# laurabragagnolo/SkelSplat

Hardware: AMD Instinct MI355X
Metric: rendered+backpropagated views/s (differentiable skeletal-Gaussian rasterizer fwd+bwd) (higher is better)
Workload: dtype f32

## Files before the change

include/skelsplat_hip.h:

```cpp
#ifndef SKELSPLAT_HIP_H
#define SKELSPLAT_HIP_H

#include <stddef.h>
#include <stdint.h>

#ifdef __cplusplus
extern "C" {
#endif

#define SKS_MAX_VIEWS 64
#define SKS_MAX_CHANNELS 32
#define SKS_SMALL_P 256

#define SKS_ANTIALIASING 1u
#define SKS_CLAMP01      2u
#define SKS_FORCE_BINNED 4u
#define SKS_DEBUG_SYNC   8u

#define SKS_NO_NT_STORES 16u

#define SKS_RAW_PARAMS   32u
#define SKS_RAW_GRADS    128u
#define SKS_BIN_CLEAN    64u
#define SKS_BIN_GROUPS_SHIFT 16
#define SKS_BIN_GROUPS(n) ((unsigned)(((n) - 1) & 7) << SKS_BIN_GROUPS_SHIFT)
#define SKS_FILL_LINEAR (1u << 21)
#define SKS_FILL_ROWS (1u << 22)
#define SKS_BWD_LDS_LIST (1u << 20)
#define SKS_BWD_WG_SHIFT 23

const char* sks_last_error(void);
int sks_version(void);

int sks_scratch_bytes(int V, int P, int C, int W, int H, size_t bin_capacity,
                      size_t* geom_bytes, size_t* binning_bytes, size_t* accum_bytes);

int sks_forward(int V, int P, int C, int W, int H,
                const float* viewmatrix, const float* projmatrix,
                const float* tanfovx , const float* tanfovy ,
                const float* means3D, const float* features, const float* opacities,
                const float* scales, const float* rotations, const float* cov3D_precomp,
                float scale_modifier, unsigned flags,
                float* out_color, float* out_invdepth, int* radii,
                void* geom, void* binning, size_t bin_capacity, int* num_rendered_dev,
                float* final_T, uint32_t* n_contrib, void* stream);

int sks_backward(int V, int P, int C, int W, int H,
                 const float* viewmatrix, const float* projmatrix,
                 const float* tanfovx , const float* tanfovy ,
                 const float* bg,
// ... 143 lines not shown
```

skelsplat_amd/_lib.py:

```python
import ctypes as C
import os

_HERE = os.path.dirname(os.path.abspath(__file__))
LIB_PATH = os.path.join(_HERE, "libskelsplat_hip.so")
_lib = None

SKS_MAX_VIEWS = 64
SKS_MAX_CHANNELS = 32
SKS_SMALL_P = 256
SKS_ANTIALIASING = 1
SKS_CLAMP01 = 2
SKS_FORCE_BINNED = 4
SKS_DEBUG_SYNC = 8
SKS_NO_NT_STORES = 16
SKS_RAW_PARAMS = 32
SKS_BIN_CLEAN = 64
SKS_RAW_GRADS = 128
SKS_FB_NO_JOIN = 1
SKS_BIN_GROUPS_SHIFT = 16
SKS_SSIM_SCRATCH_BYTES = 64 * 8


def SKS_BIN_GROUPS(n):
    return ((int(n) - 1) & 7) << SKS_BIN_GROUPS_SHIFT
# ... 32 lines not shown
    "sks_backward_fused_loss": (_i, [_i, _i, _i, _i, _i, _vp, _vp, _vp, _vp, _vp, _vp, _vp, _vp, _vp, _vp, _vp, _f, _u,
                                     _vp, _vp, _vp, _vp, _vp, _vp, _vp, _vp, _vp, _vp, _vp, _vp, _vp, _vp, _vp, _vp, _vp, _vp, _vp]),
    "sks_loop_pack_grads": (_i, [_i, _i, _vp, _vp, _vp, _vp, _vp, _vp, _vp, _vp, _vp, _vp]),
    "sks_loop_adam_step": (_i, [_i, _i, _vp, _vp, C.c_ulonglong, _i, _vp, _vp, _vp, _vp, _vp, _vp, _vp, _i, _vp, _vp, _vp,
                                _f, _vp, _i, _vp]),
    "sks_loop_adam_step_es": (_i, [_i, _i, _vp, _vp, C.c_ulonglong, _i, _vp, _vp, _vp, _vp, _vp, _vp, _vp, _i, _vp, _vp, _vp,
                                   _f, _vp, _i, _vp, _vp, _i, _f, _vp, _vp]),
    "sks_loop_shard_floats": (_sz, [_i, _i, _i]),
    "sks_adam_multi": (_i, [_i, _vp, _vp, _vp, _vp, _vp, _vp, _vp, C.c_double, C.c_double, C.c_double, _vp]),
    "sks_loop_fused_step": (_i, [_i, _i, _i, _i, _i, _vp, _vp, _vp, _vp, _vp, _f, _u, _vp, _vp, _vp, _vp, _vp, _vp, _vp,
                                 _vp, C.c_ulonglong, _i, _vp, _vp, _vp, _vp, _vp, _vp, _vp, _i, _vp, _vp, _vp, _f, _vp, _vp, _vp,
                                 _i, _vp, _vp]),
    "sks_loop_fused_step_es": (_i, [_i, _i, _i, _i, _i, _vp, _vp, _vp, _vp, _vp, _f, _u, _vp, _vp, _vp, _vp, _vp, _vp, _vp,
                                    _vp, C.c_ulonglong, _i, _vp, _vp, _vp, _vp, _vp, _vp, _vp, _i, _vp, _vp, _vp, _f, _vp, _vp,
                                    _vp, _i, _vp, _vp, _i, _f, _vp, _vp]),
    "sks_prof_enable": (_i, [_i]),
    "sks_prof_spin": (_i, [C.c_double, _vp]),
    "sks_prof_read": (_i, [_i, C.POINTER(C.c_double), C.POINTER(C.c_longlong)]),
    "sks_prof_count": (_i, [_i, C.POINTER(C.c_longlong)]),
    "sks_prof_read_quantiles": (_i, [_i, C.POINTER(C.c_double), C.POINTER(C.c_double), C.POINTER(C.c_longlong)]),
}


def load(build_if_missing=True):
    global _lib
    if _lib is not None:
        return _lib
    if build_if_missing:
        try:
            from . import build as _b
# ... 62 lines not shown
```

skelsplat_amd/csrc/sks_bwd_small.inc:

```
template <int CG>
struct BwdPix {
    float T, T_final, last_alpha, accum_inv, last_inv, dLi, bgdot;
    float dL[CG], accum_rec[CG], last_color[CG];
};

struct BwdArgs {
    int P, C, W, H;
    unsigned flags;
    Geom g;
    const float* features;
    const float* bg;
    const float* dL_color;
    const float* dL_invdepth;
    float* accum;
    const float* tile_S;
    const float* tile_N;
    const float* hm_row = nullptr;
    const float* hm_col = nullptr;
    const float* hm_cmin = nullptr;
    const float* hm_den = nullptr;
    const int* es_stop = nullptr;
    int es_stride = 0;
    int es_views = 1;
};
// ... 489 lines not shown
        for (int j = 0; j < 8; j++) grp[j] = sum[j0 + j];
        const float r = wave_sum8(grp);
        if (lane < 8) s_red[buf][wv][j0 + lane] = r;
    }
#pragma unroll
    for (int j = NV & ~7; j < NV; j++) {
        const float r = wave_sum(sum[j]);
        if (lane == 0) s_red[buf][wv][j] = r;
    }
    __syncthreads();
    if (tid < NVS)
        out[tid * BWD_SPLITS] = tid < NV ? ((s_red[buf][0][tid] + s_red[buf][1][tid]) + (s_red[buf][2][tid] + s_red[buf][3][tid])) : 0.0f;
    }
}

__global__ __launch_bounds__(256) void k_gt_tile_stats(int C, int W, int H, const float* __restrict__ gt, float* __restrict__ tile_S,
                                                        float* __restrict__ tile_N, double* __restrict__ totals)
{
    __shared__ double s_t[2][4];
    const int band = blockIdx.x, ch = blockIdx.y, v = blockIdx.z, tid = threadIdx.x;
    const int gx = (W + TILE - 1) / TILE, gy = gridDim.x;
    const size_t HW = (size_t)H * W;
    const float* plane = gt + ((size_t)v * C + ch) * HW;
    const int y0 = band * TILE, rows = min(TILE, H - y0);
    const bool vec = (W & 3) == 0;
    double tS = 0.0, tN = 0.0;
    for (int t0 = 0; t0 < gx; t0 += 64) {
        const int tx = t0 + (tid >> 2), x = tx * TILE + (tid & 3) * 4;
        float S = 0.0f, N = 0.0f;
        if (tx < gx && x < W) {
// ... 41 lines not shown
```

skelsplat_amd/csrc/sks_common.inc:

```
thread_local char g_err[512] = "";

int fail(int code, const char* fmt, ...)
{
    va_list ap;
    va_start(ap, fmt);
    vsnprintf(g_err, sizeof(g_err), fmt, ap);
    va_end(ap);
    return code;
}

#define HIP_TRY(expr)                                                                          \
    do {                                                                                       \
        hipError_t e_ = (expr);                                                                \
        if (e_ != hipSuccess) return fail((int)e_, "%s: %s", #expr, hipGetErrorString(e_));    \
    } while (0)

#define STAGE_CHECK(name)                                                                      \
    do {                                                                                       \
        HIP_TRY(hipGetLastError());                                                            \
        if (flags & SKS_DEBUG_SYNC) {                                                          \
            hipError_t e_ = hipStreamSynchronize(st);                                          \
            if (e_ != hipSuccess) return fail((int)e_, "stage %s: %s", name, hipGetErrorString(e_)); \
        }                                                                                      \
    } while (0)
// ... 121 lines not shown
inline bool cover_per_plane(int P, int W, int H, int C)
{
    return cover_enabled(P, W, H) && (C + 1) * ((H + TILE - 1) / TILE) * cover_cw(W) <= COVER_MAX_WORDS;
}
inline Geom geom_from(void* base, int V, int P, int W, int H)
{
    char* p = (char*)base;
    Geom g;
    size_t n = (size_t)V * P;
    g.co = (float4*)p; p += align256(n * sizeof(float4));
    g.xyd = (float4*)p; p += align256(n * sizeof(float4));
    g.rect = (uint4*)p; p += align256(n * sizeof(uint4));
    g.cover = cover_enabled(P, W, H) ? (uint32_t*)p : nullptr;
    return g;
}
inline size_t geom_bytes(int V, int P, int W, int H, int C)
{
    const int planes = cover_per_plane(P, W, H, C) ? C + 1 : 1;
    return 3 * align256((size_t)V * P * 16) + align256((size_t)V * planes * ((H + TILE - 1) / TILE) * cover_cw(W) * 4);
}

constexpr int BIN_WAVE_SORT = 64;
constexpr int BIN_ROWS = 2;
constexpr int BIN_CLASSES = 8;
constexpr int BIN_HDR_CLASS = 8;
constexpr int BIN_MAX_GROUPS = 7;
#ifndef SKS_BIN_FB_GROUPS
#define SKS_BIN_FB_GROUPS 1
#endif
constexpr int BIN_FB_GROUPS = SKS_BIN_FB_GROUPS;
inline int bin_groups_default()
{
    static const int n = [] {
        const char* e = getenv("SKS_BIN_GROUPS");
// ... 68 lines not shown
```

skelsplat_amd/csrc/sks_geom_bwd.inc:

```
struct GeomBwdArgs {
    int P, C, W, H;
    unsigned flags;
    const float* vms;
    const float* pms;
    const float* means;
    const float* opac;
    const float* scales;
    const float* rots;
    const float* cov3Dp;
    float smod;
    const int* radii;
    const float* accum;
    int nsplit;
    const double* gt_totals;
    double* loss_sums;
    float* packed;
    float* dmeans3D;
    float* dmeans2D;
    float* dopacity;
    float* dscales;
    float* drots;
    float* dcov3D;
    float* dfeat;
    const uint4* rect = nullptr;
    const uint32_t* goff = nullptr;
    const float* part = nullptr;
    size_t cap = 0;
    const uint32_t* bin_hdr = nullptr;
    int v0 = 0;
};

__device__ __forceinline__ float sq(float x) { return x * x; }

__device__ __forceinline__ void geom_bwd_dfeat(const GeomBwdArgs& a, size_t o0, int n, int tid, int nthreads)
{
    const int ns = a.nsplit ? a.nsplit : 1, NVS = NACC + a.C;
    for (int e = tid; e < n * a.C; e += nthreads) {
        const int gi = e / a.C, ch = e - gi * a.C;
        const float* acc = a.accum + (o0 + gi) * ns * NVS + (size_t)(NACC + ch) * ns;
        float t = 0.0f;
        if (ns == BWD_SPLITS) {
            float4 q[4];
#pragma unroll
            for (int i = 0; i < 4; i++) q[i] = reinterpret_cast<const float4*>(acc)[i];
#pragma unroll
            for (int i = 0; i < 4; i++) { t += q[i].x; t += q[i].y; t += q[i].z; t += q[i].w; }
        } else {
            for (int sp = 0; sp < ns; sp++) t += acc[sp];
        }
        a.dfeat[(o0 + gi) * a.C + ch] = t;
    }
}

template <bool DFEAT_HERE = true>
__device__ __forceinline__ void geom_bwd_load(const GeomBwdArgs& a, int v, int idx, float (&g)[NACC], double& pS, double& pN)
{
    const size_t o = (size_t)v * a.P + (idx < a.P ? idx : 0);
    const int NVS = NACC + a.C;
    const float* acc = a.accum + o * (a.nsplit ? a.nsplit : 1) * NVS;
    if (a.nsplit == BWD_SPLITS) {
        static_assert(BWD_SPLITS == 16, "4 x float4 per value");
        float4 q[NACC][4];
#pragma unroll
        for (int j = 0; j < NACC - 1; j++)
#pragma unroll
            for (int i = 0; i < 4; i++) q[j][i] = reinterpret_cast<const float4*>(acc + j * BWD_SPLITS)[i];
#pragma unroll
        for (int j = 0; j < NACC - 1; j++) {
            float t = 0.0f;
#pragma unroll
            for (int i = 0; i < 4; i++) t += (q[j][i].x + q[j][i].y) + (q[j][i].z + q[j][i].w);
            g[j] = t;
        }
        g[NACC - 1] = 0.0f;
// ... 266 lines not shown
        if (raw) {
            const float so = 1.0f / (1.0f + expf_fixed(-(PRE ? pre->opac : a.opac[idx])));
            oj = so * (1.0f - so);
        }
        pk[10] = dop * oj * scl;
    }
}

__global__ __launch_bounds__(256) void k_geom_bwd(GeomBwdArgs a, ViewTan vt)
{
    const int idx = blockIdx.x * 256 + threadIdx.x;
    const int v = blockIdx.y;
    float g[NACC];
    double pS, pN;
    if (a.dfeat) geom_bwd_dfeat(a, (size_t)v * a.P + blockIdx.x * 256, min(256, a.P - (int)blockIdx.x * 256), threadIdx.x, 256);
    geom_bwd_load<false>(a, v, idx, g, pS, pN);
    double n_view = 1.0;
    if (a.loss_sums) {
        __shared__ double s_l[2][4];
        pS = wave_sum_d(pS);
        pN = wave_sum_d(pN);
        if ((threadIdx.x & 63) == 0) { s_l[0][threadIdx.x >> 6] = pS; s_l[1][threadIdx.x >> 6] = pN; }
        __syncthreads();
        const double S = a.gt_totals[2 * v] + ((s_l[0][0] + s_l[0][1]) + (s_l[0][2] + s_l[0][3]));
        n_view = a.gt_totals[2 * v + 1] + ((s_l[1][0] + s_l[1][1]) + (s_l[1][2] + s_l[1][3]));
        if (threadIdx.x == 0) {
            a.loss_sums[2 * v] = S;
            a.loss_sums[2 * v + 1] = n_view;
        }
    }
    if (idx >= a.P) return;
// ... 55 lines not shown
        const float* acc = a.accum + o * (NACC + a.C);
        for (int ch = 0; ch < a.C; ch++) a.dfeat[o * a.C + ch] = acc[NACC + ch];
    }
    geom_bwd_finish<true>(a, vt, v, idx, g, 1.0, &in);
}

__global__ __launch_bounds__(256) void k_geom_bwd_all(GeomBwdArgs a, ViewTan vt, int V, float* __restrict__ mean_out)
{
    const int t = threadIdx.x;
    const int v = t / a.P, idx = t - v * a.P;
    const bool live = v < V;
    float g[NACC];
    double pS, pN;
    if (a.dfeat) geom_bwd_dfeat(a, 0, V * a.P, t, 256);
    if (live) {
        geom_bwd_load<false>(a, v, idx, g, pS, pN);
        geom_bwd_finish(a, vt, v, idx, g, 1.0);
    }
    __syncthreads();
    if (t < a.P) {
        float m[3] = { 0.0f, 0.0f, 0.0f };
        for (int w0 = 0; w0 < V; w0 += 4) {
            float tv[4][3];
#pragma unroll
            for (int j = 0; j < 4; j++) {
                const float* gm = a.dmeans3D + ((size_t)(w0 + j < V ? w0 + j : V - 1) * a.P + t) * 3;
                tv[j][0] = gm[0]; tv[j][1] = gm[1]; tv[j][2] = gm[2];
            }
#pragma unroll
            for (int j = 0; j < 4; j++)
                if (w0 + j < V) { m[0] += tv[j][0]; m[1] += tv[j][1]; m[2] += tv[j][2]; }
// ... 93 lines not shown
```

skelsplat_amd/csrc/sks_geom_fwd.inc:

```
__device__ __forceinline__ uint4 geom_fwd_one(int P, const ViewTan& vt, const float* __restrict__ vms,
                                              const float* __restrict__ pms, const float* __restrict__ means,
                                              const float* __restrict__ opac, const float* __restrict__ scales,
                                              const float* __restrict__ rots, const float* __restrict__ cov3Dp,
                                              float smod, unsigned flags, const Geom& g, int* __restrict__ radii,
                                              int v, int idx, bool live, bool store = true)
{
    const size_t o = (size_t)v * P + (live ? idx : 0);
    const float* V = vms + 16 * v;
    const float* PM = pms + 16 * v;
    const float tan_fovx = vt.x[v], tan_fovy = vt.y[v];
    const int W = vt.w[v], H = vt.h[v];
    const float focal_y = H / (2.0f * tan_fovy);
    const float focal_x = W / (2.0f * tan_fovx);
    const int gx = (W + TILE - 1) / TILE, gy = (H + TILE - 1) / TILE;

    int radius_out = 0;
    uint4 rect = make_uint4(0, 0, 0, 0);
    float4 co = make_float4(0, 0, 0, 0), xyd = make_float4(0, 0, 1.0f, 1.0f);

    const int li = live ? idx : 0;
    const float p_orig[3] = { means[3 * li], means[3 * li + 1], means[3 * li + 2] };
    float p_view[3];
    transformPoint4x3(p_orig, V, p_view);
    if (live && p_view[2] > 0.2f) {
// ... 36 lines not shown
                radius_out = (int)my_radius;
                rect = make_uint4(xmin, ymin, xmax, ymax);
                const float op_raw = opac[li];
                const float op = (flags & SKS_RAW_PARAMS) ? 1.0f / (1.0f + expf_fixed(-op_raw)) : op_raw;
                co = make_float4(conic[0], conic[1], conic[2], op * h_convolution_scaling);
                xyd = make_float4(px, py, p_view[2], 1 / p_view[2]);
            }
        }
    }
    if (live && store) {
        radii[o] = radius_out;
        g.co[o] = co;
        g.xyd[o] = xyd;
        g.rect[o] = rect;
    }
    return rect;
}

#ifndef SKS_GEOM_COVER_THREADS
#define SKS_GEOM_COVER_THREADS 256
#endif
__global__ __launch_bounds__(SKS_GEOM_COVER_THREADS > 256 ? SKS_GEOM_COVER_THREADS : 256) void k_geom_fwd(int P, int W, int H, ViewTan vt, const float* __restrict__ vms,
                                                   const float* __restrict__ pms, const float* __restrict__ means,
                                                   const float* __restrict__ opac, const float* __restrict__ scales,
                                                   const float* __restrict__ rots, const float* __restrict__ cov3Dp,
                                                   float smod, unsigned flags, Geom g, int* __restrict__ radii, int vf,
                                                   uint32_t* __restrict__ count = nullptr, uint32_t* __restrict__ touched = nullptr,
                                                   const float* __restrict__ features = nullptr, int C = 0,
                                                   uint2* __restrict__ fmask = nullptr, uint32_t* __restrict__ bin_hdr = nullptr,
                                                   int cover_planes = 0)
{
    __shared__ uint32_t s_cov[COVER_MAX_WORDS];
    const int idx = blockIdx.x * blockDim.x + threadIdx.x;
    const int v = blockIdx.y;
    const bool live = idx < P;
    if (vf > 0) {
        const int fr = v / vf;
        means += (size_t)fr * P * 3;
        opac += (size_t)fr * P;
        if (scales) scales += (size_t)fr * P * 3;
        if (rots) rots += (size_t)fr * P * 4;
        if (cov3Dp) cov3Dp += (size_t)fr * P * 6;
    }
    const int pz = blockIdx.z;
    const uint4 rect = geom_fwd_one(P, vt, vms, pms, means, opac, scales, rots, cov3Dp, smod, flags, g, radii, v, idx, live, pz == 0);
    if (bin_hdr && blockIdx.x == 0 && blockIdx.y == 0 && pz == 0 && threadIdx.x < 64) bin_hdr[threadIdx.x] = 0u;
    if (count) {
        const int wt = (int)(rect.z - rect.x), n = wt * (int)(rect.w - rect.y);
        if (live) touched[(size_t)v * P + idx] = (uint32_t)n;
        if (live && v == 0) {
            unsigned fm = 0u;
            float f0 = 0.0f;
            for (int ch = C - 1; ch >= 0; ch--) {
                const float f = features[(size_t)idx * C + ch];
                if (f != 0.0f) { fm |= 1u << ch; f0 = f; }
            }
            fmask[idx] = make_uint2(fm, __float_as_uint(f0));
        }
    }
    if (g.cover) {
// ... 6 lines not shown
        if (mine) {
#pragma nounroll
            for (unsigned y = rect.y; y < rect.w; y++) {
                atomicOr(&s_cov[y * cw], 1u);
#pragma nounroll
                for (unsigned w0 = rect.x >> 5; w0 <= (rect.z - 1u) >> 5; w0++) {
                    const unsigned lo = max(rect.x, w0 << 5) & 31u, hi = min(rect.z - 1u, (w0 << 5) + 31u) & 31u;
                    atomicOr(&s_cov[y * cw + 1 + w0], (0xffffffffu >> (31u - hi)) & (0xffffffffu << lo));
                }
            }
        }
        __syncthreads();
        uint32_t* out = g.cover + ((size_t)v * (cover_planes ? C + 1 : 1) + (cover_planes ? pz : 0)) * pw;
        for (int i = threadIdx.x; i < pw; i += blockDim.x) out[i] = s_cov[i];
    }
}

__global__ void k_mark_visible(int P, const float* __restrict__ means, const float* __restrict__ V,
                               uint8_t* __restrict__ present)
{
    const int idx = blockIdx.x * 256 + threadIdx.x;
    if (idx >= P) return;
    const float p[3] = { means[3 * idx], means[3 * idx + 1], means[3 * idx + 2] };
    float pv[3];
    transformPoint4x3(p, V, pv);
    present[idx] = pv[2] > 0.2f;
}
```

skelsplat_amd/csrc/sks_raster.hip:

```cpp
#include <hip/hip_runtime.h>
#include <hip/hip_ext.h>
#include <stdarg.h>
#include <stdlib.h>
#include <stdio.h>
#include <string.h>

#include "../../include/skelsplat_hip.h"
#include "sks_math.h"
#include "sks_loop_dev.h"

using namespace sks;

namespace {

#include "sks_common.inc"
#include "sks_geom_fwd.inc"
#include "sks_fwd_small.inc"
#include "sks_bwd_small.inc"
#include "sks_geom_bwd.inc"
#include "sks_binned.inc"

inline int pick_cg(int C) { return C <= 4 ? 4 : C <= 16 ? 16 : C <= 20 ? 20 : 32; }

int check_common(int V, int P, int C, int W, int H)
// ... 105 lines not shown
            case 4: hipLaunchKernelGGL((k_render_bwd_wave<4, false, true, true, ES>), grid, dim3(256), 0, st, a, vt, vo); break;
            case 16: hipLaunchKernelGGL((k_render_bwd_wave<16, false, true, true, ES>), grid, dim3(256), 0, st, a, vt, vo); break;
            case 20: hipLaunchKernelGGL((k_render_bwd_wave<20, false, true, true, ES>), grid, dim3(256), 0, st, a, vt, vo); break;
            default: hipLaunchKernelGGL((k_render_bwd_wave<32, false, true, true, ES>), grid, dim3(256), 0, st, a, vt, vo); break;
        }
        return;
    }
    switch (cg) {
        case 4: hipLaunchKernelGGL((k_render_bwd_wave<4, false, true, false, ES>), grid, dim3(256), 0, st, a, vt, vo); break;
        case 16: hipLaunchKernelGGL((k_render_bwd_wave<16, false, true, false, ES>), grid, dim3(256), 0, st, a, vt, vo); break;
        case 20: hipLaunchKernelGGL((k_render_bwd_wave<20, false, true, false, ES>), grid, dim3(256), 0, st, a, vt, vo); break;
        default: hipLaunchKernelGGL((k_render_bwd_wave<32, false, true, false, ES>), grid, dim3(256), 0, st, a, vt, vo); break;
    }
}

template <int CG>
void launch_bwd_small(const BwdArgs& a, const ViewTan& vt, const ViewOff& vo, int V, int gy, bool dfeat, hipStream_t st,
                      const ProfScope& prof)
{
    (void)gy;
    if (a.P <= 64 && !(a.flags & (1u << 20))) {
        dim3 grid(a.P, V, bwd_wave_groups(V, a.P, a.flags));
        if (dfeat) SKS_LAUNCH(prof, (k_render_bwd_wave<CG, true, false>), grid, dim3(256), 0, st, a, vt, vo);
        else SKS_LAUNCH(prof, (k_render_bwd_wave<CG, false, false>), grid, dim3(256), 0, st, a, vt, vo);
        return;
    }
    dim3 grid(a.P, V, BWD_SPLITS);
    const size_t lds = GatherLds<CG>::bytes((a.P + 15) & ~15, CG, a.C);
    if (lds > 48 * 1024) {
        (void)hipFuncSetAttribute(reinterpret_cast<const void*>(&k_render_bwd_gather<CG, true>),
                                  hipFuncAttributeMaxDynamicSharedMemorySize, (int)lds);
        (void)hipFuncSetAttribute(reinterpret_cast<const void*>(&k_render_bwd_gather<CG, false>),
                                  hipFuncAttributeMaxDynamicSharedMemorySize, (int)lds);
    }
    if (dfeat) SKS_LAUNCH(prof, (k_render_bwd_gather<CG, true>), grid, dim3(256), lds, st, a);
// ... 46 lines not shown
}

}

#ifndef SKS_GEOM_BINNED_THREADS
#define SKS_GEOM_BINNED_THREADS 256
#endif

extern "C" {

const char* sks_last_error(void) { return g_err; }
void sks_set_error_(const char* msg)
{
    snprintf(g_err, sizeof(g_err), "%s", msg);
}
int sks_version(void) { return 12; }

int sks_scratch_bytes(int V, int P, int C, int W, int H, size_t bin_capacity, size_t* geom, size_t* binning, size_t* accum)
{
    if (int rc = check_common(V, P, C, W, H)) return rc;
    const int NT = ((W + TILE - 1) / TILE) * ((H + TILE - 1) / TILE);
    if (geom) *geom = geom_bytes(V, P > 0 ? P : 1, W, H, C);
    if (binning) *binning = bin_bytes(V, P, NT, bin_capacity, C + 1, (size_t)((H + TILE - 1) / TILE) * cover_cw(W));
    if (accum) *accum = (size_t)V * (P > 0 ? P : 1) * BWD_SPLITS * (NACC + C) * sizeof(float);
    return 0;
}

}

namespace {

int forward_impl(int V, int P, int C, int W, int H, const float* viewmatrix, const float* projmatrix,
                 const float* tanfovx, const float* tanfovy, const float* means3D, const float* features,
                 const float* opacities, const float* scales, const float* rotations, const float* cov3D_precomp,
                 float scale_modifier, unsigned flags, float* out_color, float* out_invdepth, int* radii, void* geom,
                 void* binning, size_t bin_capacity, int* num_rendered_dev, float* final_T, uint32_t* n_contrib,
                 void* stream, const FwdHook* hook)
{
    if (int rc = check_common(V, P, C, W, H)) return rc;
    hipStream_t st = (hipStream_t)stream;
// ... 18 lines not shown

    const bool small = P <= SKS_SMALL_P && !(flags & SKS_FORCE_BINNED);
    Bin b{};
    if (!small) {
        if (!binning) return fail(-2, "binned path needs a binning buffer");
        if (bin_capacity < 1) return fail(-1, "binned path needs bin_capacity >= 1");
        b = bin_from(binning, V, P, NT, bin_capacity);
    }
    if (!small) g.cover = nullptr;
    const int gthreads = small ? 256 : SKS_GEOM_BINNED_THREADS;
    const int gplanes = (small && g.cover && cover_per_plane(P, W, H, C)) ? C + 1 : 1;
    if (hook && small && hook->geom_done)
        hipExtLaunchKernelGGL(k_geom_fwd, dim3((P + gthreads - 1) / gthreads, V, gplanes), dim3(gthreads), 0, st, nullptr, hook->geom_done, 0,
                              P, W, H, vt, viewmatrix, projmatrix, means3D, opacities, scales, rotations, cov3D_precomp, scale_modifier,
                              flags, g, radii, 0, (uint32_t*)nullptr, (uint32_t*)nullptr, features, C, (uint2*)nullptr, (uint32_t*)nullptr,
                              cover_per_plane(P, W, H, C) ? 1 : 0);
    else
    hipLaunchKernelGGL(k_geom_fwd, dim3((P + gthreads - 1) / gthreads, V, gplanes), dim3(gthreads), 0, st, P, W, H, vt, viewmatrix, projmatrix,
                       means3D, opacities, scales, rotations, cov3D_precomp, scale_modifier, flags, g, radii, 0,
                       small ? (uint32_t*)nullptr : b.count, small ? (uint32_t*)nullptr : b.touched, features, C,
                       small ? (uint2*)nullptr : b.fmask, small ? (uint32_t*)nullptr : b.hdr, (small && cover_per_plane(P, W, H, C)) ? 1 : 0);
    STAGE_CHECK("geometry");
    if (hook && small && hook->after_geom) {
        if (int rc = hook->after_geom(hook->ctx)) return rc;
    }

    FwdArgs a{ P, C, W, H, flags, g, features, out_color, out_invdepth, final_T, n_contrib, composite_slots(flags, V, P),
               ((1u << 20) + (unsigned)C) / (unsigned)(C + 1), 0, (!small || (g.cover && cover_per_plane(P, W, H, C))) ? 1 : 0,
               (W >= 2 && W < 16384) ? (unsigned)(((1ull << 32) + (unsigned)W - 1) / (unsigned)W) : 0u };
    const int cg = pick_cg(C);
    if (small) {
        {
            ProfScope prof(0, st, true);
            switch (cg) {
                case 4: launch_fwd_small<4>(a, V, gy, st, prof); break;
                case 16: launch_fwd_small<16>(a, V, gy, st, prof); break;
// ... 84 lines not shown
    if (P == 0) return 0;
    hipStream_t st = (hipStream_t)stream;
    if (!viewmatrix || !projmatrix || !tanfovx || !tanfovy || !means3D || !features || !opacities || !radii ||
        !geom || !dL_dout_color || !accum || !dL_dmeans3D || !dL_dmeans2D || !dL_dopacity)
        return fail(-2, "missing required pointer");
    if (!cov3D_precomp && (!scales || !rotations)) return fail(-2, "need scales+rotations or cov3D_precomp");
    ViewTan vt;
    ViewOff vo;
    fill_views(vt, &vo, V, C, W, H, tanfovx, tanfovy, nullptr, nullptr);
    Geom g = geom_from(const_cast<void*>(geom), V, P, W, H);
    const int gx = (W + TILE - 1) / TILE, gy = (H + TILE - 1) / TILE, NT = gx * gy;
    BwdArgs a{ P, C, W, H, flags, g, features, bg, dL_dout_color, dL_dout_invdepth, (float*)accum, nullptr, nullptr };
    const int cg = pick_cg(C);
    const bool dfeat = dL_dfeatures != nullptr;
    const bool small = P <= SKS_SMALL_P && !(flags & SKS_FORCE_BINNED);
    int vg = V, ng = 1;
    if (!small) bin_groups(flags, V, vg, ng);
    if (group >= ng) return fail(-1, "view group %d of %d", group, ng);
    if ((phases & BWD_RENDER) && small) {
        ProfScope prof(1, st, true);
        switch (cg) {
            case 4: launch_bwd_small<4>(a, vt, vo, V, gy, dfeat, st, prof); break;
            case 16: launch_bwd_small<16>(a, vt, vo, V, gy, dfeat, st, prof); break;
            case 20: launch_bwd_small<20>(a, vt, vo, V, gy, dfeat, st, prof); break;
            default: launch_bwd_small<32>(a, vt, vo, V, gy, dfeat, st, prof); break;
        }
        STAGE_CHECK("render-backward(small)");
    } else if (phases & BWD_RENDER) {
        if (!binning) return fail(-2, "binned path needs the forward's binning buffer");
        Bin b = bin_from(const_cast<void*>(binning), V, P, NT, bin_capacity);
        BinView bv = bin_view(b, NT, bin_capacity);
        if (dfeat && group <= 0) HIP_TRY(hipMemsetAsync(accum, 0, (size_t)V * P * (NACC + C) * sizeof(float), st));
        dim3 grid(bwd_tile_blocks());
        const unsigned magic_nt = (unsigned)(((1ull << 32) + (unsigned)NT - 1) / (unsigned)NT), magic_gx = (unsigned)(((1ull << 32) + (unsigned)gx - 1) / (unsigned)gx);
        const bool extra = bg != nullptr || dL_dout_invdepth != nullptr;
        for (int gi = group < 0 ? 0 : group; gi < (group < 0 ? ng : group + 1); gi++) {
            const uint4* tl = b.tlist + (size_t)gi * vg * NT;
            const uint32_t* hd = b.hdr + gi * BIN_CLASSES;
            ProfScope prof(1, st);
            if (dfeat) hipLaunchKernelGGL((k_render_bwd_tile<true, true>), grid, dim3(BWD_TILE_THREADS), 0, st, a, bv, gx, V, magic_nt, magic_gx, tl, hd);
            else if (extra) hipLaunchKernelGGL((k_render_bwd_tile<false, true>), grid, dim3(BWD_TILE_THREADS), 0, st, a, bv, gx, V, magic_nt, magic_gx, tl, hd);
            else hipLaunchKernelGGL((k_render_bwd_tile<false, false>), grid, dim3(BWD_TILE_THREADS), 0, st, a, bv, gx, V, magic_nt, magic_gx, tl, hd);
        }
        STAGE_CHECK("render-backward(binned)");
    }
    if (!(phases & BWD_GEOM)) return 0;
    GeomBwdArgs ga{ P, C, W, H, flags, viewmatrix, projmatrix, means3D, opacities, scales, rotations, cov3D_precomp,
                    scale_modifier, radii, (const float*)accum, small ? BWD_SPLITS : 0, nullptr, nullptr, nullptr, dL_dmeans3D, dL_dmeans2D, dL_dopacity, dL_dscales,
                    dL_drotations, dL_dcov3D, dL_dfeatures };
    if (!small) {
        Bin b = bin_from(const_cast<void*>(binning), V, P, NT, bin_capacity);
        ga.rect = g.rect;
        ga.goff = b.goff;
        ga.part = b.part;
        ga.cap = bin_capacity;
        ga.bin_hdr = b.hdr;
    }
    if (dL_dmeans3D_mean && V * P <= 256 && small) {
        hipLaunchKernelGGL(k_geom_bwd_all, dim3(1), dim3(256), 0, st, ga, vt, V, dL_dmeans3D_mean);
    } else {
        if (small) hipLaunchKernelGGL(k_geom_bwd, dim3((P + 255) / 256, V), dim3(256), 0, st, ga, vt);
        else {
            const int v0 = group < 0 ? 0 : group * vg, nv = group < 0 ? V : ((V - v0 < vg) ? V - v0 : vg);
            ga.v0 = v0;
// ... 189 lines not shown
{
    if (int rc = check_common(V, P, C, W, H)) return rc;
    if (P < 1) return fail(-1, "P must be positive");
    if (frames < 1 || V % frames) return fail(-1, "frames must divide the number of views (V = %d, frames = %d)", V, frames);
    if (!viewmatrix || !projmatrix || !tanfovx || !tanfovy || !means3D || !opacities || !radii || !geom)
        return fail(-2, "missing required pointer");
    if (!cov3D_precomp && (!scales || !rotations)) return fail(-2, "need scales+rotations or cov3D_precomp");
    hipStream_t st = (hipStream_t)stream;
    ViewTan vt;
    if (!fill_views(vt, nullptr, V, C, W, H, tanfovx, tanfovy, view_wh, nullptr))
        return fail(-1, "view_wh: every view's size must be within [1, W] x [1, H] (pass the largest as W, H)");
    Geom g = geom_from(geom, V, P, W, H);
    g.cover = nullptr;
    hipLaunchKernelGGL(k_geom_fwd, dim3((P + 255) / 256, V), dim3(256), 0, st, P, W, H, vt, viewmatrix, projmatrix,
                       means3D, opacities, scales, rotations, cov3D_precomp, scale_modifier, flags, g, radii,
                       frames > 1 ? V / frames : 0);
    STAGE_CHECK("geometry");
    return 0;
}

static int loop_fused_step_impl(int V, int P, int C, int W, int H, const float* viewmatrix, const float* projmatrix,
                                const float* tanfovx, const float* tanfovy, const float* features, float scale_modifier,
                                unsigned flags, int* radii, void* geom, const float* gt, const double* gt_totals, void* accum,
                                double* loss_sums, float* packed, float* slots, unsigned long long group_mask, int last_view,
                                float* xyz, float* scaling, float* rotation, float* opacity, float* exp_avg, float* exp_avg_sq,
                                int* counters, int acc_steps, const double* lr_sched, const double* lrs, const double* adam,
                                float lambda_consistency, const int* limb, const int* view_wh, const size_t* gt_offsets,
                                int frames, const float* const* hm_factors, int* es_state, int es_window, float es_tolerance,
                                int* es_host_flags, void* stream)
{
    if (int rc = check_common(V, P, C, W, H)) return rc;
// ... 184 lines not shown
```

Baseline: 60380.

## Add task-list backward render kernel with depth-sorted per-view compact Gaussian data

Geometry forward now emits, per view, a depth-sorted compact copy of each visible Gaussian's conic, position, rect and id, plus a flat list of (gaussian, split slot) tasks. A new backward render kernel walks this task list with a grid sized from a host-mapped hint of the previous call's task count. Each task writes its own accumulator row, so the render backward skips culled or empty work and avoids atomics. Geometry backward reduces the per-split rows in the new layout. The scheme adds scratch memory, couples the launch grid to data from an earlier call, and adds a pinned host buffer.

```diff
diff --git a/include/skelsplat_hip.h b/include/skelsplat_hip.h
--- a/include/skelsplat_hip.h
+++ b/include/skelsplat_hip.h
@@ -34,6 +34,7 @@
 
 int sks_scratch_bytes(int V, int P, int C, int W, int H, size_t bin_capacity,
                       size_t* geom_bytes, size_t* binning_bytes, size_t* accum_bytes);
+int sks_bwd_task_grid(int workgroups);
 
 int sks_forward(int V, int P, int C, int W, int H,
                 const float* viewmatrix, const float* projmatrix,
diff --git a/skelsplat_amd/_lib.py b/skelsplat_amd/_lib.py
--- a/skelsplat_amd/_lib.py
+++ b/skelsplat_amd/_lib.py
@@ -70,6 +70,7 @@
     "sks_loop_fused_step_es": (_i, [_i, _i, _i, _i, _i, _vp, _vp, _vp, _vp, _vp, _f, _u, _vp, _vp, _vp, _vp, _vp, _vp, _vp,
                                     _vp, C.c_ulonglong, _i, _vp, _vp, _vp, _vp, _vp, _vp, _vp, _i, _vp, _vp, _vp, _f, _vp, _vp,
                                     _vp, _i, _vp, _vp, _i, _f, _vp, _vp]),
+    "sks_bwd_task_grid": (_i, [_i]),
     "sks_prof_enable": (_i, [_i]),
     "sks_prof_spin": (_i, [C.c_double, _vp]),
     "sks_prof_read": (_i, [_i, C.POINTER(C.c_double), C.POINTER(C.c_longlong)]),
diff --git a/skelsplat_amd/csrc/sks_bwd_small.inc b/skelsplat_amd/csrc/sks_bwd_small.inc
--- a/skelsplat_amd/csrc/sks_bwd_small.inc
+++ b/skelsplat_amd/csrc/sks_bwd_small.inc
@@ -527,6 +527,218 @@
     }
 }
 
+template <int CG, bool DFEAT>
+__global__ __launch_bounds__(256, (DFEAT || CG > 20) ? 1 : 4) void k_render_bwd_task(BwdArgs a, ViewTan vt, ViewOff vo, BwdTasks tk,
+                                                                                     uint32_t* __restrict__ hint)
+{
+    constexpr int NV = NACC + (DFEAT ? CG : 0);
+    __shared__ float s_red[2][4][NV];
+    const int v = blockIdx.y, tid = threadIdx.x, lane = tid & 63, wv = tid >> 6;
+    const int P = a.P, C = a.C, W = vt.w[v], H = vt.h[v];
+    const int NW = DFEAT ? NACC + C : NACC;
+    const size_t HW = (size_t)H * W;
+    const size_t go = (size_t)v * P;
+    const float* dL_view = a.dL_color + vo.off[v];
+    const uint32_t* tasks = tk.task + go * BWD_SPLITS;
+    const uint32_t ntask = tk.count[v];
+    uint32_t t0 = tasks[blockIdx.x];
+    const bool has = lane < P;
+    const int li = has ? lane : 0;
+    const float4 m_co = tk.co[go + li];
+    const float4 m_xyd = tk.xyd[go + li];
+    uint4 m_rect = tk.rect[go + li];
+    if (!has) m_rect = make_uint4(0, 0, 0, 0);
+    const unsigned m_id = tk.id[go + li];
+    float m_feat[CG];
+    unsigned m_fmask = 0;
+#pragma unroll
+    for (int ch = 0; ch < CG; ch++) {
+        m_feat[ch] = (ch < C && has) ? a.features[li * C + ch] : 0.0f;
+        m_fmask |= m_feat[ch] != 0.0f ? (1u << ch) : 0u;
+    }
+    if (hint && blockIdx.x == 0 && tid == 0) hint[v] = ntask + 1u;
+    const unsigned chmask = (C >= 32 ? 0xffffffffu : ((1u << C) - 1u));
+    const bool do_clamp = a.flags & SKS_CLAMP01;
+    const float ddelx_dx = (float)(0.5 * W), ddely_dy = (float)(0.5 * H);
+    const unsigned chmask_all = chmask;
+    const size_t HW_all = HW;
+    float* const frows = a.accum + (size_t)gridDim.y * P * BWD_SPLITS * NACC;
+    int buf = 0;
+    for (uint32_t j = blockIdx.x; j < ntask; j += gridDim.x) {
+    if (j != blockIdx.x) t0 = tasks[j];
+    const int g = (int)(t0 & 0xffu), slot = (int)((t0 >> 8) & 0xffu), kg = (int)(t0 >> 16);
+    const unsigned gx0 = rlu(m_rect.x, kg), gy0 = rlu(m_rect.y, kg), gx1 = rlu(m_rect.z, kg), gy1 = rlu(m_rect.w, kg);
+    const int wt = (int)gx1 - (int)gx0, ht = (int)gy1 - (int)gy0;
+    const int nchunks = wt * ht;
+    const int nslot = nchunks < BWD_SPLITS ? nchunks : BWD_SPLITS;
+    if (slot == BWD_SPLITS || slot == nslot - 1) {
+        const int z0 = slot == BWD_SPLITS ? 0 : nslot;
+        const size_t r0 = (go + g) * BWD_SPLITS + z0;
+        if (tid < (BWD_SPLITS - z0) * NACC) a.accum[r0 * NACC + tid] = 0.0f;
+        if (DFEAT)
+            for (int i = tid; i < (BWD_SPLITS - z0) * C; i += 256) frows[r0 * C + i] = 0.0f;
+        if (slot == BWD_SPLITS) continue;
+    }
+    float sum[NV];
+#pragma unroll
+    for (int jj = 0; jj < NV; jj++) sum[jj] = 0.0f;
+    for (int c = slot; c < nchunks; c += BWD_SPLITS) {
+        unsigned chmask = chmask_all;
+        size_t HW = HW_all;
+        asm volatile("" : "+s"(chmask), "+s"(HW));
+        const int tyl = c / wt;
+        const int tx = (int)gx0 + (c - tyl * wt), ty = (int)gy0 + tyl;
+        const int x = tx * TILE + (tid & 15), y = ty * TILE + (tid >> 4);
+        const bool in = x < W && y < H;
+        const float pxf = (float)x, pyf = (float)y;
+        const bool hitc = !((unsigned)tx < m_rect.x || (unsigned)tx >= m_rect.z || (unsigned)ty < m_rect.y || (unsigned)ty >= m_rect.w);
+        const unsigned long long covm = __ballot(hitc);
+        float T = 1.0f, col[CG];
+#pragma unroll
+        for (int ch = 0; ch < CG; ch++) col[ch] = 0.0f;
+        int klast = -1;
+        bool alive = in;
+        unsigned chm_t = (DFEAT || a.bg != nullptr) ? chmask : 0u;
+        for (unsigned long long m = covm; m; m &= m - 1) {
+            if (!__any(alive)) break;
+            const int lk = __builtin_ctzll(m);
+            const int gk = (int)rlu(m_id, lk);
+            const unsigned fmk = rlu(m_fmask, gk);
+            chm_t |= chmask & fmk;
+            const float ex = rl(m_xyd.x, lk), ey = rl(m_xyd.y, lk);
+            const float cx = rl(m_co.x, lk), cy = rl(m_co.y, lk), cz = rl(m_co.z, lk), cw = rl(m_co.w, lk);
+            const bool cov = alive;
+            const float dx = ex - pxf, dy = ey - pyf;
+            const float power = -0.5f * (cx * dx * dx + cz * dy * dy) - cy * dx * dy;
+            const float alpha = fminf(0.99f, cw * expf_fixed(power));
+            const float test_T = T * (1 - alpha);
+            const bool pass = cov && !(power > 0.0f) && !(alpha < 1.0f / 255.0f);
+            const bool stop = pass && test_T < 0.0001f;
+            const bool acc = pass && !stop;
+            if (do_clamp) {
+                for (unsigned fm = chmask & fmk; fm; fm &= fm - 1) {
+                    const int ch = __builtin_ctz(fm);
+                    const float f = rl(m_feat[ch], gk);
+                    const float add = f * alpha * T;
+                    col[ch] += acc ? add : 0.0f;
+                }
+            }
+            if (acc) { T = test_T; klast = lk; }
+            if (stop) alive = false;
+        }
+        const bool need = in && klast >= kg;
+        if (!__any(need)) continue;
+        const size_t pix = (size_t)y * W + x;
+        struct { float T, T_final, last_alpha, accum_inv, last_inv, bgdot, dLi; } s;
+        s.T = T; s.T_final = T; s.last_alpha = 0; s.accum_inv = 0; s.last_inv = 0; s.bgdot = 0;
+        s.dLi = (need && a.dL_invdepth) ? a.dL_invdepth[(size_t)v * HW + pix] : 0.0f;
+        {
+            const float* dLc = dL_view + pix;
+            for (unsigned fm = chm_t; fm;) {
+                int cc[4];
+                float cv[4], gv[4];
+#pragma unroll
+                for (int i = 0; i < 4; i++) {
+                    cc[i] = fm ? __builtin_ctz(fm) : -1;
+                    fm &= fm - 1;
+                }
+#pragma unroll
+                for (int i = 0; i < 4; i++) cv[i] = col[max(cc[i], 0)];
+#pragma unroll
+                for (int i = 0; i < 4; i++) gv[i] = (cc[i] >= 0 && need) ? dLc[(size_t)max(cc[i], 0) * HW] : 0.0f;
+#pragma unroll
+                for (int i = 0; i < 4; i++) {
+                    if (cc[i] < 0) break;
+                    const int ch = cc[i];
+                    float d = gv[i];
+                    if (do_clamp && !(cv[i] >= 0.0f && cv[i] <= 1.0f)) d = 0.0f;
+                    if (a.bg) s.bgdot += a.bg[ch] * d;
+                    col[ch] = d;
+                }
+            }
+        }
+        float rec_dot = 0.0f, last_dot = 0.0f;
+        for (unsigned long long m = covm & (~0ull << kg); m; m &= ~(1ull << (63 - __builtin_clzll(m)))) {
+            const int lk = 63 - __builtin_clzll(m);
+            const bool cand = need && lk <= klast;
+            if (!__any(cand)) continue;
+            const int gk = (int)rlu(m_id, lk);
+            const float ex = rl(m_xyd.x, lk), ey = rl(m_xyd.y, lk), einvd = rl(m_xyd.w, lk);
+            const float cx = rl(m_co.x, lk), cy = rl(m_co.y, lk), cz = rl(m_co.z, lk), cw = rl(m_co.w, lk);
+            const float dx = ex - pxf, dy = ey - pyf;
+            const float power = -0.5f * (cx * dx * dx + cz * dy * dy) - cy * dx * dy;
+            const float G = expf_fixed(power);
+            const float alpha = fminf(0.99f, cw * G);
+            const bool act = cand && !(power > 0.0f) && !(alpha < 1.0f / 255.0f);
+            if (!__any(act)) continue;
+            const bool mine = lk == kg;
+            float Tn = s.T, dchannel_dcolor = 0.0f, dL_dalpha = 0.0f;
+            if (act) {
+                Tn = s.T / (1.f - alpha);
+                dchannel_dcolor = alpha * Tn;
+            }
+            float cdot = 0.0f;
+            for (unsigned fm = chmask & rlu(m_fmask, gk); fm; fm &= fm - 1) {
+                const int ch = __builtin_ctz(fm);
+                cdot += rl(m_feat[ch], gk) * col[ch];
+            }
+            if (DFEAT && mine) {
+#pragma unroll
+                for (int ch = 0; ch < CG; ch++) {
+                    if ((chmask & (1u << ch)) && act) sum[NACC + ch] += dchannel_dcolor * col[ch];
+                }
+            }
+            if (act) {
+                rec_dot = s.last_alpha * last_dot + (1.f - s.last_alpha) * rec_dot;
+                last_dot = cdot;
+                dL_dalpha += cdot - rec_dot;
+                s.T = Tn;
+                s.accum_inv = s.last_alpha * s.last_inv + (1.f - s.last_alpha) * s.accum_inv;
+                s.last_inv = einvd;
+                dL_dalpha += (einvd - s.accum_inv) * s.dLi;
+                dL_dalpha *= s.T;
+                s.last_alpha = alpha;
+                dL_dalpha += (-s.T_final / (1.f - alpha)) * s.bgdot;
+                if (mine) {
+                    const float dL_dG = cw * dL_dalpha;
+                    const float gdx = G * dx, gdy = G * dy;
+                    const float dG_ddelx = -gdx * cx - gdy * cy;
+                    const float dG_ddely = -gdy * cz - gdx * cy;
+                    sum[0] += dL_dG * dG_ddelx * ddelx_dx;
+                    sum[1] += dL_dG * dG_ddely * ddely_dy;
+                    sum[2] += -0.5f * gdx * dx * dL_dG;
+                    sum[3] += -0.5f * gdx * dy * dL_dG;
+                    sum[4] += -0.5f * gdy * dy * dL_dG;
+                    sum[5] += G * dL_dalpha;
+                    sum[6] += dchannel_dcolor * s.dLi;
+                }
+            }
+        }
+    }
+#pragma unroll
+    for (int j0 = 0; j0 + 8 <= NV; j0 += 8) {
+        float grp[8];
+#pragma unroll
+        for (int jj = 0; jj < 8; jj++) grp[jj] = sum[j0 + jj];
+        const float r = wave_sum8(grp);
+        if (lane < 8) s_red[buf][wv][j0 + lane] = r;
+    }
+#pragma unroll
+    for (int jj = NV & ~7; jj < NV; jj++) {
+        const float r = wave_sum(sum[jj]);
+        if (lane == 0) s_red[buf][wv][jj] = r;
+    }
+    __syncthreads();
+    if (tid < NW) {
+        const size_t row = (go + g) * BWD_SPLITS + slot;
+        const float r = (s_red[buf][0][tid] + s_red[buf][1][tid]) + (s_red[buf][2][tid] + s_red[buf][3][tid]);
+        if (tid < NACC) a.accum[row * NACC + tid] = r;
+        else frows[row * C + (tid - NACC)] = r;
+    }
+    buf ^= 1;
+    }
+}
+
 __global__ __launch_bounds__(256) void k_gt_tile_stats(int C, int W, int H, const float* __restrict__ gt, float* __restrict__ tile_S,
                                                         float* __restrict__ tile_N, double* __restrict__ totals)
 {
diff --git a/skelsplat_amd/csrc/sks_common.inc b/skelsplat_amd/csrc/sks_common.inc
--- a/skelsplat_amd/csrc/sks_common.inc
+++ b/skelsplat_amd/csrc/sks_common.inc
@@ -159,10 +159,40 @@
     g.cover = cover_enabled(P, W, H) ? (uint32_t*)p : nullptr;
     return g;
 }
-inline size_t geom_bytes(int V, int P, int W, int H, int C)
+constexpr int BWD_TASK_MAX_P = 64;
+constexpr int BWD_TASK_MAX_PAIRS = 256;
+inline bool bwd_tasks_enabled(int V, int P) { return P >= 1 && P <= BWD_TASK_MAX_P && V * P <= BWD_TASK_MAX_PAIRS; }
+struct BwdTasks {
+    uint32_t* count;
+    uint32_t* task;
+    float4* co;
+    float4* xyd;
+    uint4* rect;
+    uint32_t* id;
+};
+inline size_t geom_base_bytes(int V, int P, int W, int H, int C)
 {
     const int planes = cover_per_plane(P, W, H, C) ? C + 1 : 1;
     return 3 * align256((size_t)V * P * 16) + align256((size_t)V * planes * ((H + TILE - 1) / TILE) * cover_cw(W) * 4);
+}
+inline size_t task_bytes(int V, int P)
+{
+    if (!bwd_tasks_enabled(V, P)) return 0;
+    return align256((size_t)V * 4) + align256((size_t)V * P * BWD_SPLITS * 4) + 3 * align256((size_t)V * P * 16) + align256((size_t)V * P * 4);
+}
+inline size_t geom_bytes(int V, int P, int W, int H, int C) { return geom_base_bytes(V, P, W, H, C) + task_bytes(V, P); }
+inline BwdTasks tasks_from(void* base, int V, int P, int W, int H, int C)
+{
+    BwdTasks t{};
+    if (!bwd_tasks_enabled(V, P)) return t;
+    char* p = (char*)base + geom_base_bytes(V, P, W, H, C);
+    t.count = (uint32_t*)p; p += align256((size_t)V * 4);
+    t.task = (uint32_t*)p; p += align256((size_t)V * P * BWD_SPLITS * 4);
+    t.co = (float4*)p; p += align256((size_t)V * P * 16);
+    t.xyd = (float4*)p; p += align256((size_t)V * P * 16);
+    t.rect = (uint4*)p; p += align256((size_t)V * P * 16);
+    t.id = (uint32_t*)p;
+    return t;
 }
 
 constexpr int BIN_WAVE_SORT = 64;
diff --git a/skelsplat_amd/csrc/sks_geom_bwd.inc b/skelsplat_amd/csrc/sks_geom_bwd.inc
--- a/skelsplat_amd/csrc/sks_geom_bwd.inc
+++ b/skelsplat_amd/csrc/sks_geom_bwd.inc
@@ -28,7 +28,10 @@
     size_t cap = 0;
     const uint32_t* bin_hdr = nullptr;
     int v0 = 0;
+    bool trows = false;
+    size_t tfeat = 0;
 };
+
 
 __device__ __forceinline__ float sq(float x) { return x * x; }
 
@@ -39,7 +42,14 @@
         const int gi = e / a.C, ch = e - gi * a.C;
         const float* acc = a.accum + (o0 + gi) * ns * NVS + (size_t)(NACC + ch) * ns;
         float t = 0.0f;
-        if (ns == BWD_SPLITS) {
+        if (a.trows) {
+            const float* row = a.accum + a.tfeat + (o0 + gi) * BWD_SPLITS * a.C + ch;
+            float q[BWD_SPLITS];
+#pragma unroll
+            for (int sp = 0; sp < BWD_SPLITS; sp++) q[sp] = row[sp * a.C];
+#pragma unroll
+            for (int sp = 0; sp < BWD_SPLITS; sp++) t += q[sp];
+        } else if (ns == BWD_SPLITS) {
             float4 q[4];
 #pragma unroll
             for (int i = 0; i < 4; i++) q[i] = reinterpret_cast<const float4*>(acc)[i];
@@ -52,12 +62,31 @@
     }
 }
 
-template <bool DFEAT_HERE = true>
+template <bool DFEAT_HERE = true, bool TASK_ROWS = false>
 __device__ __forceinline__ void geom_bwd_load(const GeomBwdArgs& a, int v, int idx, float (&g)[NACC], double& pS, double& pN)
 {
     const size_t o = (size_t)v * a.P + (idx < a.P ? idx : 0);
     const int NVS = NACC + a.C;
     const float* acc = a.accum + o * (a.nsplit ? a.nsplit : 1) * NVS;
+    if (TASK_ROWS && a.trows) {
+        const float4* row = reinterpret_cast<const float4*>(a.accum + o * BWD_SPLITS * NACC);
+        float4 q[BWD_SPLITS][2];
+#pragma unroll
+        for (int sp = 0; sp < BWD_SPLITS; sp++) { q[sp][0] = row[2 * sp]; q[sp][1] = row[2 * sp + 1]; }
+#pragma unroll
+        for (int j = 0; j < NACC - 1; j++) {
+            const auto val = [&](int sp) { const float4 x = q[sp][j >> 2]; return (j & 3) == 0 ? x.x : ((j & 3) == 1 ? x.y : ((j & 3) == 2 ? x.z : x.w)); };
+            float t = 0.0f;
+#pragma unroll
+            for (int i = 0; i < 4; i++) t += (val(4 * i) + val(4 * i + 1)) + (val(4 * i + 2) + val(4 * i + 3));
+            g[j] = t;
+        }
+        g[NACC - 1] = 0.0f;
+        if (DFEAT_HERE && a.dfeat) geom_bwd_dfeat(a, o, 1, 0, 1);
+        pS = 0.0;
+        pN = 0.0;
+        return;
+    }
     if (a.nsplit == BWD_SPLITS) {
         static_assert(BWD_SPLITS == 16, "4 x float4 per value");
         float4 q[NACC][4];
@@ -354,7 +383,7 @@
     float g[NACC];
     double pS, pN;
     if (a.dfeat) geom_bwd_dfeat(a, (size_t)v * a.P + blockIdx.x * 256, min(256, a.P - (int)blockIdx.x * 256), threadIdx.x, 256);
-    geom_bwd_load<false>(a, v, idx, g, pS, pN);
+    geom_bwd_load<false, true>(a, v, idx, g, pS, pN);
     double n_view = 1.0;
     if (a.loss_sums) {
         __shared__ double s_l[2][4];
@@ -440,7 +469,7 @@
     double pS, pN;
     if (a.dfeat) geom_bwd_dfeat(a, 0, V * a.P, t, 256);
     if (live) {
-        geom_bwd_load<false>(a, v, idx, g, pS, pN);
+        geom_bwd_load<false, true>(a, v, idx, g, pS, pN);
         geom_bwd_finish(a, vt, v, idx, g, 1.0);
     }
     __syncthreads();
diff --git a/skelsplat_amd/csrc/sks_geom_fwd.inc b/skelsplat_amd/csrc/sks_geom_fwd.inc
--- a/skelsplat_amd/csrc/sks_geom_fwd.inc
+++ b/skelsplat_amd/csrc/sks_geom_fwd.inc
@@ -3,7 +3,8 @@
                                               const float* __restrict__ opac, const float* __restrict__ scales,
                                               const float* __restrict__ rots, const float* __restrict__ cov3Dp,
                                               float smod, unsigned flags, const Geom& g, int* __restrict__ radii,
-                                              int v, int idx, bool live, bool store = true)
+                                              int v, int idx, bool live, bool store = true, float4* co_out = nullptr,
+                                              float4* xyd_out = nullptr)
 {
     const size_t o = (size_t)v * P + (live ? idx : 0);
     const float* V = vms + 16 * v;
@@ -74,6 +75,7 @@
         g.xyd[o] = xyd;
         g.rect[o] = rect;
     }
+    if (co_out) { *co_out = co; *xyd_out = xyd; }
     return rect;
 }
 
@@ -88,7 +90,7 @@
                                                    uint32_t* __restrict__ count = nullptr, uint32_t* __restrict__ touched = nullptr,
                                                    const float* __restrict__ features = nullptr, int C = 0,
                                                    uint2* __restrict__ fmask = nullptr, uint32_t* __restrict__ bin_hdr = nullptr,
-                                                   int cover_planes = 0)
+                                                   int cover_planes = 0, BwdTasks tk = {})
 {
     __shared__ uint32_t s_cov[COVER_MAX_WORDS];
     const int idx = blockIdx.x * blockDim.x + threadIdx.x;
@@ -103,7 +105,21 @@
         if (cov3Dp) cov3Dp += (size_t)fr * P * 6;
     }
     const int pz = blockIdx.z;
-    const uint4 rect = geom_fwd_one(P, vt, vms, pms, means, opac, scales, rots, cov3Dp, smod, flags, g, radii, v, idx, live, pz == 0);
+    float4 co, xyd;
+    const uint4 rect = geom_fwd_one(P, vt, vms, pms, means, opac, scales, rots, cov3Dp, smod, flags, g, radii, v, idx, live, pz == 0, &co, &xyd);
+    const bool tk_here = tk.task && pz == (gridDim.z > 1 ? 1 : 0) && threadIdx.x < 64;
+    unsigned tk_pos = 0, tk_off = 0, tk_n = 0;
+    if (tk_here) {
+        const unsigned depth = __float_as_uint(xyd.z);
+        const unsigned nt = (rect.z - rect.x) * (rect.w - rect.y);
+        tk_n = nt == 0 ? 1u : (nt < (unsigned)BWD_SPLITS ? nt : (unsigned)BWD_SPLITS);
+        for (int j = 0; j < P; j++) {
+            const unsigned dj = (unsigned)__builtin_amdgcn_readlane((int)depth, j);
+            const unsigned nj = (unsigned)__builtin_amdgcn_readlane((int)tk_n, j);
+            tk_pos += (dj < depth || (dj == depth && j < idx)) ? 1u : 0u;
+            tk_off += j < idx ? nj : 0u;
+        }
+    }
     if (bin_hdr && blockIdx.x == 0 && blockIdx.y == 0 && pz == 0 && threadIdx.x < 64) bin_hdr[threadIdx.x] = 0u;
     if (count) {
         const int wt = (int)(rect.z - rect.x), n = wt * (int)(rect.w - rect.y);
@@ -140,6 +156,17 @@
         uint32_t* out = g.cover + ((size_t)v * (cover_planes ? C + 1 : 1) + (cover_planes ? pz : 0)) * pw;
         for (int i = threadIdx.x; i < pw; i += blockDim.x) out[i] = s_cov[i];
     }
+    if (tk_here && live) {
+        const size_t so = (size_t)v * P + tk_pos;
+        tk.co[so] = co;
+        tk.xyd[so] = xyd;
+        tk.rect[so] = rect;
+        tk.id[so] = (uint32_t)idx;
+        uint32_t* tl = tk.task + (size_t)v * P * BWD_SPLITS + tk_off;
+        const bool culled = rect.z == rect.x;
+        for (unsigned s = 0; s < tk_n; s++) tl[s] = (uint32_t)idx | ((culled ? (unsigned)BWD_SPLITS : s) << 8) | (tk_pos << 16);
+        if (idx == P - 1) tk.count[v] = tk_off + tk_n;
+    }
 }
 
 __global__ void k_mark_visible(int P, const float* __restrict__ means, const float* __restrict__ V,
diff --git a/skelsplat_amd/csrc/sks_raster.hip b/skelsplat_amd/csrc/sks_raster.hip
--- a/skelsplat_amd/csrc/sks_raster.hip
+++ b/skelsplat_amd/csrc/sks_raster.hip
@@ -143,11 +143,56 @@
     }
 }
 
+struct TaskHint {
+    uint32_t* h[16] = {};
+    int grid = 0;
+};
+thread_local TaskHint tl_task_hint;
+uint32_t* task_hint_buf(hipStream_t st)
+{
+    int dev = 0;
+    if (hipGetDevice(&dev) != hipSuccess || dev < 0 || dev >= 16) return nullptr;
+    uint32_t*& h = tl_task_hint.h[dev];
+    if (!h) {
+        hipStreamCaptureStatus cs = hipStreamCaptureStatusNone;
+        if (hipStreamIsCapturing(st, &cs) != hipSuccess || cs != hipStreamCaptureStatusNone) return nullptr;
+        void* p = nullptr;
+        if (hipHostMalloc(&p, SKS_MAX_VIEWS * sizeof(uint32_t), hipHostMallocPortable | hipHostMallocMapped) != hipSuccess) return nullptr;
+        memset(p, 0, SKS_MAX_VIEWS * sizeof(uint32_t));
+        h = (uint32_t*)p;
+    }
+    return h;
+}
+int task_grid(const uint32_t* hint, int V, int P)
+{
+    const int bound = P * BWD_SPLITS;
+    int n = tl_task_hint.grid;
+    if (n <= 0) {
+        unsigned m = 0;
+        for (int v = 0; v < V && hint; v++) {
+            const unsigned h = ((volatile const uint32_t*)hint)[v];
+            if (h == 0) { m = 0; break; }
+            m = h - 1 > m ? h - 1 : m;
+        }
+        n = (hint && m > 0) ? (int)(m + m / 8 + 1) : bound;
+    }
+    return n < 1 ? 1 : (n > bound ? bound : n);
+}
+
 template <int CG>
 void launch_bwd_small(const BwdArgs& a, const ViewTan& vt, const ViewOff& vo, int V, int gy, bool dfeat, hipStream_t st,
-                      const ProfScope& prof)
+                      const ProfScope& prof, const BwdTasks& tk)
 {
     (void)gy;
+    if (tk.task) {
+        static const int env = [] { const char* e = getenv("SKS_BWD_TASK_GRID"); return e ? atoi(e) : 0; }();
+        if (env > 0 && tl_task_hint.grid <= 0) tl_task_hint.grid = env;
+        uint32_t* hint = env > 0 ? nullptr : task_hint_buf(st);
+        const dim3 grid(task_grid(hint, V, a.P), V);
+        if (dfeat) SKS_LAUNCH(prof, (k_render_bwd_task<CG, true>), grid, dim3(256), 0, st, a, vt, vo, tk, hint);
+        else SKS_LAUNCH(prof, (k_render_bwd_task<CG, false>), grid, dim3(256), 0, st, a, vt, vo, tk, hint);
+        return;
+    }
     if (a.P <= 64 && !(a.flags & (1u << 20))) {
         dim3 grid(a.P, V, bwd_wave_groups(V, a.P, a.flags));
         if (dfeat) SKS_LAUNCH(prof, (k_render_bwd_wave<CG, true, false>), grid, dim3(256), 0, st, a, vt, vo);
@@ -224,7 +269,7 @@
 {
     snprintf(g_err, sizeof(g_err), "%s", msg);
 }
-int sks_version(void) { return 12; }
+int sks_version(void) { return 13; }
 
 int sks_scratch_bytes(int V, int P, int C, int W, int H, size_t bin_capacity, size_t* geom, size_t* binning, size_t* accum)
 {
@@ -234,6 +279,13 @@
     if (binning) *binning = bin_bytes(V, P, NT, bin_capacity, C + 1, (size_t)((H + TILE - 1) / TILE) * cover_cw(W));
     if (accum) *accum = (size_t)V * (P > 0 ? P : 1) * BWD_SPLITS * (NACC + C) * sizeof(float);
     return 0;
+}
+
+int sks_bwd_task_grid(int workgroups)
+{
+    const int prev = tl_task_hint.grid;
+    tl_task_hint.grid = workgroups > 0 ? workgroups : 0;
+    return prev;
 }
 
 }
@@ -282,12 +334,13 @@
         hipExtLaunchKernelGGL(k_geom_fwd, dim3((P + gthreads - 1) / gthreads, V, gplanes), dim3(gthreads), 0, st, nullptr, hook->geom_done, 0,
                               P, W, H, vt, viewmatrix, projmatrix, means3D, opacities, scales, rotations, cov3D_precomp, scale_modifier,
                               flags, g, radii, 0, (uint32_t*)nullptr, (uint32_t*)nullptr, features, C, (uint2*)nullptr, (uint32_t*)nullptr,
-                              cover_per_plane(P, W, H, C) ? 1 : 0);
+                              cover_per_plane(P, W, H, C) ? 1 : 0, tasks_from(geom, V, P, W, H, C));
     else
     hipLaunchKernelGGL(k_geom_fwd, dim3((P + gthreads - 1) / gthreads, V, gplanes), dim3(gthreads), 0, st, P, W, H, vt, viewmatrix, projmatrix,
                        means3D, opacities, scales, rotations, cov3D_precomp, scale_modifier, flags, g, radii, 0,
                        small ? (uint32_t*)nullptr : b.count, small ? (uint32_t*)nullptr : b.touched, features, C,
-                       small ? (uint2*)nullptr : b.fmask, small ? (uint32_t*)nullptr : b.hdr, (small && cover_per_plane(P, W, H, C)) ? 1 : 0);
+                       small ? (uint2*)nullptr : b.fmask, small ? (uint32_t*)nullptr : b.hdr, (small && cover_per_plane(P, W, H, C)) ? 1 : 0,
+                       small ? tasks_from(geom, V, P, W, H, C) : BwdTasks{});
     STAGE_CHECK("geometry");
     if (hook && small && hook->after_geom) {
         if (int rc = hook->after_geom(hook->ctx)) return rc;
@@ -402,16 +455,17 @@
     const int cg = pick_cg(C);
     const bool dfeat = dL_dfeatures != nullptr;
     const bool small = P <= SKS_SMALL_P && !(flags & SKS_FORCE_BINNED);
+    const BwdTasks tk = (small && !(flags & SKS_BWD_LDS_LIST)) ? tasks_from(const_cast<void*>(geom), V, P, W, H, C) : BwdTasks{};
     int vg = V, ng = 1;
     if (!small) bin_groups(flags, V, vg, ng);
     if (group >= ng) return fail(-1, "view group %d of %d", group, ng);
     if ((phases & BWD_RENDER) && small) {
         ProfScope prof(1, st, true);
         switch (cg) {
-            case 4: launch_bwd_small<4>(a, vt, vo, V, gy, dfeat, st, prof); break;
-            case 16: launch_bwd_small<16>(a, vt, vo, V, gy, dfeat, st, prof); break;
-            case 20: launch_bwd_small<20>(a, vt, vo, V, gy, dfeat, st, prof); break;
-            default: launch_bwd_small<32>(a, vt, vo, V, gy, dfeat, st, prof); break;
+            case 4: launch_bwd_small<4>(a, vt, vo, V, gy, dfeat, st, prof, tk); break;
+            case 16: launch_bwd_small<16>(a, vt, vo, V, gy, dfeat, st, prof, tk); break;
+            case 20: launch_bwd_small<20>(a, vt, vo, V, gy, dfeat, st, prof, tk); break;
+            default: launch_bwd_small<32>(a, vt, vo, V, gy, dfeat, st, prof, tk); break;
         }
         STAGE_CHECK("render-backward(small)");
     } else if (phases & BWD_RENDER) {
@@ -436,6 +490,10 @@
     GeomBwdArgs ga{ P, C, W, H, flags, viewmatrix, projmatrix, means3D, opacities, scales, rotations, cov3D_precomp,
                     scale_modifier, radii, (const float*)accum, small ? BWD_SPLITS : 0, nullptr, nullptr, nullptr, dL_dmeans3D, dL_dmeans2D, dL_dopacity, dL_dscales,
                     dL_drotations, dL_dcov3D, dL_dfeatures };
+    if (tk.task) {
+        ga.trows = true;
+        ga.tfeat = (size_t)V * P * BWD_SPLITS * NACC;
+    }
     if (!small) {
         Bin b = bin_from(const_cast<void*>(binning), V, P, NT, bin_capacity);
         ga.rect = g.rect;
@@ -655,7 +713,8 @@
     g.cover = nullptr;
     hipLaunchKernelGGL(k_geom_fwd, dim3((P + 255) / 256, V), dim3(256), 0, st, P, W, H, vt, viewmatrix, projmatrix,
                        means3D, opacities, scales, rotations, cov3D_precomp, scale_modifier, flags, g, radii,
-                       frames > 1 ? V / frames : 0);
+                       frames > 1 ? V / frames : 0, (uint32_t*)nullptr, (uint32_t*)nullptr, (const float*)nullptr, C, (uint2*)nullptr,
+                       (uint32_t*)nullptr, 0, (P <= SKS_SMALL_P && !(flags & SKS_FORCE_BINNED)) ? tasks_from(geom, V, P, W, H, C) : BwdTasks{});
     STAGE_CHECK("geometry");
     return 0;
 }
```

Result: no change. 60800 (median of 6 runs) (+0.7%).
